# pmelchior/scarlet

Measured on AMD Instinct MI355X. Metric: PGM iters/sec over batched blends; achieved HBM GB/s vs roofline, higher is better.
Workload: dtype f32; 1 GPU; configs[2]: 1024 independent 5-band 128x128 blends in total, 10 ExtendedSource components (41x41) each, ConvolutionRenderer FFT 160x160; iterations 0..1234 of a fit from the initial parameters; loop=blend, blends_total=1024, components_per_blend=10, sub_ranges_per_gpu=3

## Files before the change

scarlet_amd/batch.py:

```python

import collections
import ctypes

import numpy as np

from . import _lib, operator


MonotonicPlanes = collections.namedtuple("MonotonicPlanes", "center_radius variance max_iter")
MonotonicPlanes.__doc__ = """The constraint of the coefficients of ``StarletMorphology(monotonic=True)`` as the device
runs it: ``MonotonicMaskConstraint((h // 2, w // 2), center_radius, variance, max_iter)`` on
every plane.  Given to ``ComponentSpec(starlet=(coefficients, MonotonicPlanes(...)))`` in the
place of the thresholds."""


def monotonic_planes_prox(stack, rule=MonotonicPlanes(1, 0.0, 3)):
    out = np.array(stack, dtype=np.float32, order="C")
    assert out.ndim == 3
    planes, h, w = out.shape
    _lib.check(_lib.load().smi_starlet_monotonic_mask_f32(
        _lib.ptr(out, ctypes.c_float), planes, h, w, int(rule.center_radius),
        float(rule.variance), int(rule.max_iter)))
    return out

# ... 547 lines not shown
        return a.value, e.value

    def states(self):
        out = np.zeros(self.n_blends, dtype=np.int32)
        _lib.check(self._lib.smi_batch_get_states(self._h, _lib.ptr(out, ctypes.c_int32)))
        return out

    def fit(self, max_iter=200, e_rel=1e-3, min_iter=1, prox_max_iter=10, sync_every=10):
        if max_iter > self.max_iter:
            raise ValueError("max_iter exceeds the loss-history capacity of this batch")
        n_iter = np.zeros(self.n_blends, dtype=np.int32)
        _lib.check(
            self._lib.smi_batch_fit(
                self._h, max_iter, e_rel, min_iter, prox_max_iter, sync_every,
                _lib.ptr(n_iter, ctypes.c_int32),
            )
        )
        loss = self.loss_history()
        last = np.array([loss[b][n_iter[b] - 1] if n_iter[b] else np.nan
                         for b in range(self.n_blends)])
        return n_iter, -last

    def loss_history(self):
        out = np.empty((self.n_blends, self.max_iter), dtype=np.float64)
        n = np.zeros(self.n_blends, dtype=np.int32)
        _lib.check(
            self._lib.smi_batch_get_loss(
                self._h, _lib.ptr(out, ctypes.c_double), self.max_iter,
                _lib.ptr(n, ctypes.c_int32),
            )
        )
        return [out[b, : min(n[b], self.max_iter)].copy() for b in range(self.n_blends)]

    def set_previous_loss(self, loss):
        loss = np.ascontiguousarray(np.broadcast_to(loss, (self.n_blends,)), dtype=np.float64)
        _lib.check(self._lib.smi_batch_set_previous_loss(self._h, _lib.ptr(loss, ctypes.c_double)))

    def add_observation(self, data, weights, kernel):
        data, weights, kernel = _lib.f32(data), _lib.f32(weights), _lib.f32(kernel)
        assert data.shape == weights.shape == (self.n_blends, self.C, self.H, self.W)
        assert kernel.shape == self._kernel_shape, "kernel stamp shape is fixed at construction"
        _lib.check(self._lib.smi_batch_add_observation(
            self._h, _lib.ptr(data, ctypes.c_float), _lib.ptr(weights, ctypes.c_float),
            _lib.ptr(kernel, ctypes.c_float)))

    def add_loss_constant(self, constant):
        c = np.ascontiguousarray(np.broadcast_to(constant, (self.n_blends,)), dtype=np.float64)
        _lib.check(self._lib.smi_batch_add_loss_constant(self._h, _lib.ptr(c, ctypes.c_double)))

    def set_sub_ranges(self, n):
        _lib.check(self._lib.smi_batch_set_sub_ranges(self._h, int(n)))

    def set_inline_render(self, on):
        _lib.check(self._lib.smi_batch_set_inline_render(self._h, int(bool(on))))

    def sub_ranges(self):
        n = ctypes.c_int32()
        _lib.check(self._lib.smi_batch_get_sub_ranges(self._h, ctypes.byref(n)))
        return n.value

    def attach_lowres(self, resampler, channels, data, weights, log_norm):
        channels = np.ascontiguousarray(channels, dtype=np.int32)
        data = np.ascontiguousarray(data, dtype=np.float32)
        weights = np.ascontiguousarray(weights, dtype=np.float32)
        assert data.shape == weights.shape and data.shape[0] == len(channels)
        self._lowres_shapes = getattr(self, "_lowres_shapes", []) + [data.shape]
        _lib.check(self._lib.smi_batch_attach_lowres(
            self._h, resampler, _lib.ptr(channels, ctypes.c_int32),
            _lib.ptr(data, ctypes.c_float), _lib.ptr(weights, ctypes.c_float), float(log_norm)))

    def lowres_rendered(self, index=0):
        out = np.empty(self._lowres_shapes[index], dtype=np.float32)
        _lib.check(self._lib.smi_batch_get_lowres_rendered(self._h, index,
                                                           _lib.ptr(out, ctypes.c_float)))
        return out

    def reset(self):
        _lib.check(self._lib.smi_batch_reset(self._h))

    def save_state(self):
        _lib.check(self._lib.smi_batch_save_state(self._h))

    def restore_state(self):
        _lib.check(self._lib.smi_batch_restore_state(self._h))

    def parameters(self):
        sed = np.empty((self.n_components, self.C), dtype=np.float32)
        morph = np.empty(int(self._morph_offsets[-1]), dtype=np.float32)
        _lib.check(
            self._lib.smi_batch_get_parameters(
                self._h, _lib.ptr(sed, ctypes.c_float), _lib.ptr(morph, ctypes.c_float)
            )
        )
        return sed, self._split_morphs(morph)

    def _split_starlets(self, flat):
        out, pos = [], 0
        for shape in self._star_shapes:
            n = int(np.prod(shape))
            out.append(flat[pos:pos + n].reshape(shape))
            pos += n
        return out

    def starlet_state(self, dtype=np.float32):
        n = int(sum(np.prod(s) for s in self._star_shapes))
        names = ("coeffs", "m", "v", "vhat", "gradient")
        bufs = [np.zeros(n, dtype=np.float32) for _ in names]
# ... 132 lines not shown
```

scarlet_amd/csrc/batch.hip:

```cpp
#include <rocfft/rocfft.h>

#include <algorithm>
#include <cmath>
#include <cstdlib>
#include <atomic>
#include <cstring>
#include <limits>
#include <map>
#include <mutex>
#include <thread>
#include <tuple>
#include <utility>

#include "common.h"

namespace smi {

static thread_local std::string g_error;
static std::atomic<int> g_hw_queues{4};
static std::atomic<long long> g_observation_uploads{0};
static std::mutex g_plan_mutex;
void set_error(const std::string &msg) { g_error = msg; }

static int next_fast_len(int n) {
// ... 101 lines not shown
    auto it = g_live_shapes.find(std::make_tuple(device, Fy, Fx));
    if (it != g_live_shapes.end() && --it->second <= 0) g_live_shapes.erase(it);
}

static int plans_get(int device, int Fy, int Fx, int count, bool shared, PlanPair *out) {
    if (!shared) return make_plans(Fy, Fx, count, out);
    std::lock_guard<std::mutex> guard(g_plan_mutex);
    PlanPair &p = g_plan_cache[device].by_count[count];
    if (!p.fwd) {
        const int rc = make_plans(Fy, Fx, count, &p);
        if (rc) return rc;
    }
    *out = p;
    return SMI_OK;
}

struct smi_batch {
    smi_batch_desc d{};
    int device = 0;
    hipStream_t stream = nullptr;
    bool null_renderer = false;
    bool fused = false;
    int Fy = 0, Fx = 0, Fxh = 0;
    int Py = 0, Px = 0;
    float2 *Kt = nullptr;
    long long *dbg = nullptr;
    float *P = nullptr, *Q = nullptr;
    float2 *S = nullptr, *Khat = nullptr;
    void *work = nullptr;
    rocfft_plan plan_fwd = nullptr, plan_inv = nullptr;
    bool plans_registered = false, plans_shared = false;
    rocfft_execution_info info = nullptr;
    float *data = nullptr, *weights = nullptr;
    float4 *dw = nullptr;
    bool own_obs = false;
    double *log_norm = nullptr;
    int32_t *comp_start = nullptr, *c_blend = nullptr, *c_oy = nullptr, *c_ox = nullptr,
            *c_h = nullptr, *c_w = nullptr, *c_flags = nullptr, *c_plan = nullptr;
    int64_t *c_moff = nullptr;
    float *c_sed_min_step = nullptr, *c_sed_rel = nullptr, *c_morph_step = nullptr,
          *c_morph_rel = nullptr, *c_min_grad = nullptr, *c_lthresh = nullptr;
    float *sed = nullptr, *morph = nullptr;
    float *mom[6] = {nullptr, nullptr, nullptr, nullptr, nullptr, nullptr};
    float *g_sed = nullptr, *g_morph = nullptr;
    float *xp_tmp = nullptr;
    int n_size_classes = 0;
    double *pt = nullptr, *g_center = nullptr;
    float *c_sigma = nullptr, *c_beta = nullptr;
    int n_point = 0;
    std::vector<double> box_center;
    std::vector<char> is_point;
    int n_shift = 0, max_box_side = 1, max_box_w = 1;
    float *shift_scratch = nullptr;
    bool inline_render = true;
    float *morph_param = nullptr, *c_shift_step = nullptr, *c_shift_rel = nullptr;
    int32_t *c_shift_fft = nullptr;
    std::vector<char> is_shift;
    smi::StarletView star{};
    int32_t *st_comp = nullptr, *st_planes = nullptr, *st_fixed = nullptr, *st_toff = nullptr;
    int64_t *st_coff = nullptr;
    float *st_thresh = nullptr, *st_coeffs = nullptr, *st_mom[3] = {nullptr, nullptr, nullptr},
          *st_grad = nullptr, *st_work = nullptr;
    int64_t n_star_coeffs = 0;
    int32_t *st_mono = nullptr, *st_mono_radius = nullptr, *st_mono_iter = nullptr;
    double *st_mono_var = nullptr;
    float *st_zsave = nullptr;
    smi::ProfileView prof{};
    int32_t *pf_comp = nullptr, *pf_kind = nullptr, *pf_fixed = nullptr;
    double *pf_step = nullptr, *pf_rel = nullptr, *pf_par = nullptr, *pf_grad = nullptr,
           *pf_mom[3] = {nullptr, nullptr, nullptr};
    std::vector<int64_t> h_moff;
    std::vector<int32_t> h_blend;
    float *c_center_floor = nullptr, *c_bg_level = nullptr, *c_fista_step = nullptr;
    float *c_sym_strength = nullptr;
    int32_t *c_chain_repeat = nullptr;
    int32_t mono_mask = 0;
    float *c_pos_floor = nullptr, *c_sed_floor = nullptr;
    double *fista_t = nullptr;
    smi::KernelShiftView ks{};
    float *ks_resid = nullptr;
    double2 *ks_tmp = nullptr;
    void *saved[12] = {};
    size_t saved_bytes[12] = {};
    int scheme = SMI_SCHEME_AMSGRAD;
    bool include_log_norm = true;
    bool lite_flags = false;
    int32_t *have_prev = nullptr;
    float *scratch = nullptr;
    int64_t n_morph = 0;
    bool have_components = false, have_obs = false, have_kernel = false;
    std::vector<smi::LowRes *> lowres;
    double *extra_terms = nullptr;
    int n_sub = 0;
    std::vector<int32_t> h_comp_start;
    struct ObsLayer {
        float *data = nullptr, *weights = nullptr;
        float2 *Kt = nullptr;
        float4 *dw = nullptr;
    };
    std::vector<ObsLayer> layers;
    float *Q2 = nullptr;
    int32_t *work_items = nullptr;
    int32_t stage_plan[kNumUpdateClasses];
    std::vector<int32_t> h_work_start;
    std::vector<hipStream_t> sub_streams;
    std::vector<hipEvent_t> sub_events;
    int32_t *state = nullptr, *zero_state = nullptr, *n_loss = nullptr, *status_out = nullptr;
    int32_t *it_base = nullptr;
    int32_t *frame_hw = nullptr;
    int32_t *pause_at = nullptr, *conv_flag = nullptr;
    std::vector<char> plan_shared;
    int32_t *h_round = nullptr;
    double *loss_hist = nullptr, *last_loss = nullptr, *loss_partial = nullptr;
    std::vector<SweepPlanDev> plans;
    SweepPlanDev *d_plans = nullptr;
    int max_levels = 0;
    BatchView view{};
    float b1 = 0.9f, b2 = 0.999f, eps = 1e-8f;
    double b1_f64 = 0.9, b2_f64 = 0.999;
    bool timing = false;
    std::vector<hipEvent_t> events;
    double phase_ms[6] = {0, 0, 0, 0, 0, 0};
    int timed_iters = 0;
};

namespace {

void refresh_view(smi_batch *b) {
    BatchView &v = b->view;
    v.nb = b->d.n_blends;
    v.C = b->d.C;
    v.H = b->d.H;
    v.W = b->d.W;
    v.Fy = b->Py;
    v.Fx = b->Px;
    v.n_comp = b->d.n_components;
    v.n_comp_total = b->d.n_components;
    v.comp_start = b->comp_start;
    v.c_blend = b->c_blend;
    v.c_oy = b->c_oy;
    v.c_ox = b->c_ox;
    v.c_h = b->c_h;
    v.c_w = b->c_w;
    v.c_flags = b->c_flags;
    v.c_plan = b->c_plan;
    v.c_moff = b->c_moff;
    v.c_sed_min_step = b->c_sed_min_step;
    v.c_sed_rel = b->c_sed_rel;
    v.c_morph_step = b->c_morph_step;
    v.c_morph_rel = b->c_morph_rel;
    v.c_min_grad = b->c_min_grad;
    v.c_lthresh = b->c_lthresh;
    v.sed = b->sed;
    v.morph = b->morph;
    v.m_sed = b->mom[0];
    v.v_sed = b->mom[1];
    v.vh_sed = b->mom[2];
    v.m_morph = b->mom[3];
    v.v_morph = b->mom[4];
    v.vh_morph = b->mom[5];
    v.data = b->data;
    v.weights = b->weights;
    v.dw = b->dw;
    v.it_base = b->it_base;
    v.frame_hw = b->frame_hw;
    v.pause_at = b->pause_at;
    v.conv_flag = b->conv_flag;
    v.log_norm = b->log_norm;
    v.state = b->state;
    v.n_loss = b->n_loss;
    v.loss_hist = b->loss_hist;
    v.hist_cap = b->d.max_iter;
    v.last_loss = b->last_loss;
    v.have_prev = b->have_prev;
    v.scratch = b->scratch;
    v.loss_partial = b->loss_partial;
    v.n_partial = b->fused ? b->d.C * (1 + (int)b->layers.size()) : (b->d.H * b->d.W + 255) / 256;
    v.plans = b->d_plans;
    v.max_levels = b->max_levels;
    v.fast_plans = 1;
    v.mono_mask = b->mono_mask;
    v.b1 = b->b1;
    v.b2 = b->b2;
    v.eps = b->eps;
    v.n_point = b->n_point;
    v.pt = b->pt;
    v.c_sigma = b->c_sigma;
    v.c_beta = b->c_beta;
    v.n_shift = b->n_shift;
    v.max_box_side = b->max_box_side;
    v.shift_scratch = b->shift_scratch;
    v.morph_param = b->morph_param;
    v.g_sed_buf = b->g_sed;
    v.g_morph_buf = b->g_morph;
    v.xp_tmp = b->xp_tmp;
    v.n_morph_total = b->n_morph;
    v.c_shift_step = b->c_shift_step;
    v.c_shift_rel = b->c_shift_rel;
    v.c_shift_fft = b->c_shift_fft;
    v.c_center_floor = b->c_center_floor;
    v.c_sym_strength = b->c_sym_strength;
    v.c_chain_repeat = b->c_chain_repeat;
    v.c_pos_floor = b->c_pos_floor;
    v.c_sed_floor = b->c_sed_floor;
    v.c_bg_level = b->c_bg_level;
    v.scheme = b->scheme;
    v.lite = b->scheme == SMI_SCHEME_FISTA || b->lite_flags;
    v.c_fista_step = b->c_fista_step;
    v.fista_t = b->fista_t;
    v.extra_term = b->extra_terms;
    v.n_extra = (int32_t)b->lowres.size();
    v.blend0 = 0;
    v.comp0 = 0;
    v.work = b->work_items;
    v.work0 = 0;
    v.work_start = b->h_work_start.data();
    v.nb_total = b->d.n_blends;
    for (int cls = 0; cls < kNumUpdateClasses; ++cls) {
        const int p = b->have_components ? b->stage_plan[cls] : -1;
        static const bool may_late = [] {
            const char *e = getenv("SMI_RING_LATE");
            return !e || atoi(e) != 0;
        }();
        const bool ok = p >= 0 && p < (int)b->plans.size() && b->plans[p].ring &&
                        kUpdateTeam[cls] == 64 && b->plans[p].ring_planes == 1 &&
                        (may_late || b->plans[p].ring_nat == b->plans[p].ring_pad);
        v.stage_plan[cls] = ok ? p : -1;
        v.stage_bytes[cls] = ok ? b->plans[p].ring_bytes : 0;
    }
    {
        const int slots = (b->max_box_w + 14) / 16 + 1;
        v.render_slots = slots <= 6 ? slots : 0;
    }
    for (const auto &pl : b->plans)
        if (!pl.slots) v.fast_plans = 0;
}

int ready(smi_batch *b) {
    SMI_REQUIRE(b != nullptr, "null batch");
    SMI_REQUIRE(b->have_components, "smi_batch_set_components has not been called");
    SMI_REQUIRE(b->have_obs, "smi_batch_set_observation has not been called");
    SMI_REQUIRE(b->null_renderer || b->have_kernel, "smi_batch_set_kernel has not been called");
    SMI_HIP(hipSetDevice(b->device));
    return SMI_OK;
}

int fft_exec(smi_batch *b, rocfft_plan plan, void *in, void *out) {
    void *ins[1] = {in}, *outs[1] = {out};
    SMI_FFT(rocfft_execute(plan, ins, outs, b->info));
    return SMI_OK;
}

int convolve(smi_batch *b, const BatchView &v, int conj) {
    if (b->null_renderer) return SMI_OK;
    if (b->fused) {
        set_error("internal: rocFFT convolution requested on the fused path");
        return SMI_ERR_INVALID;
    }
    int rc = fft_exec(b, b->plan_fwd, b->P, b->S);
    if (rc) return rc;
    launch_cmul(b->S, b->Khat, v.nb, v.C, (int64_t)b->Fy * b->Fxh, b->d.kernel_bands,
                b->d.kernel_per_blend, conj, v.state, b->stream);
    return fft_exec(b, b->plan_inv, b->S, b->Q);
}

BatchView unmasked_view(smi_batch *b) {
    BatchView v = b->view;
    v.state = b->zero_state;
    return v;
}

int upload_plans(smi_batch *b) {
    if (b->d_plans) {
        SMI_HIP(hipFree(b->d_plans));
        b->d_plans = nullptr;
    }
    if (!b->plans.empty()) {
        SMI_HIP(dev_alloc(&b->d_plans, b->plans.size()));
        SMI_HIP(hipMemcpy(b->d_plans, b->plans.data(), b->plans.size() * sizeof(SweepPlanDev),
                          hipMemcpyHostToDevice));
    }
    refresh_view(b);
    return SMI_OK;
}

// ... 2094 lines not shown
        }
    }
    SMI_HIP(hipGetLastError());
    return SMI_OK;
}

int smi_batch_gradient(smi_batch *b, float *g_sed, float *g_morph) {
    int rc = ready(b);
    if (rc) return rc;
    const BatchView v = unmasked_view(b);
    if (b->fused) {
        launch_render(v, b->P, b->stream);
        if ((rc = lowres_evaluate_all(b, 1))) return rc;
        if (b->ks.stamp && (rc = kernel_shift_backward(b, v, 0, 1))) return rc;
        if ((rc = launch_fused_conv(v, b->Fy, b->Fx, b->P, b->Kt, b->d.kernel_bands,
                                    b->d.kernel_per_blend, b->Q, 0, b->dbg, b->stream)))
            return rc;
        if ((rc = layers_evaluate(b, v, 1, b->stream))) return rc;
    } else {
        launch_render(v, b->P, b->stream);
        if ((rc = lowres_evaluate_all(b, 1))) return rc;
        if ((rc = convolve(b, v, 0))) return rc;
        launch_residual(v, b->Q, b->P, b->stream);
        if ((rc = convolve(b, v, 1))) return rc;
    }
    lowres_add_all(b);
    if ((rc = launch_update(v, b->Q, 0, 0.f, 0, b->g_sed, b->g_morph, 1, b->stream))) return rc;
    if ((rc = launch_point_sources(v, b->Q, 0, 0.f, 0, b->g_sed, b->g_center, 1, b->stream)))
        return rc;
    if ((rc = launch_shift_backward(v, b->Q, 0, b->g_center, 1, b->stream))) return rc;
    if ((rc = launch_starlet_step(v, b->star, b->Q, 0, 0.f, 0, 1, b->stream))) return rc;
    if ((rc = launch_profile_step(v, b->prof, b->Q, 0, 0.f, 0, 1, b->stream))) return rc;
    SMI_HIP(hipStreamSynchronize(b->stream));
    if (g_sed)
        SMI_HIP(hipMemcpy(g_sed, b->g_sed, (size_t)v.n_comp * v.C * sizeof(float),
                          hipMemcpyDeviceToHost));
    if (g_morph)
        SMI_HIP(hipMemcpy(g_morph, b->g_morph, (size_t)b->n_morph * sizeof(float),
                          hipMemcpyDeviceToHost));
    SMI_HIP(hipGetLastError());
    return SMI_OK;
}

static bool plain_batch(const smi_batch *b) {
    return b->fused && b->n_point == 0 && b->n_shift == 0 && b->star.n_star == 0 && b->prof.n_prof == 0 &&
           b->lowres.empty() && b->layers.empty() && !b->ks.stamp;
}

static bool inline_render(const smi_batch *b) {
    static const bool allowed = [] {
        const char *e = getenv("SMI_INLINE_RENDER");
        return !(e && e[0] == '0');
    }();
    return allowed && b->inline_render && b->fused && b->lowres.empty() && b->layers.empty() &&
           !b->ks.stamp && b->star.n_star == 0 && b->prof.n_prof == 0 && b->view.render_slots > 0;
}


static bool class_streams_pay(const smi_batch *b) {
    static const int forced = [] {
        const char *e = getenv("SMI_RANGE_CLASS_STREAMS");
        return e ? atoi(e) : -1;
    }();
    if (forced == 0 || b->n_size_classes < 2) return false;
    if (forced > 0) return true;
    return g_hw_queues.load(std::memory_order_relaxed) >= 8 && b->d.n_components >= 10000;
}

static int sub_ranges(const smi_batch *b) {
    if (!plain_batch(b)) return 1;
    const int nb = b->d.n_blends;
    const int queues = g_hw_queues.load(std::memory_order_relaxed);
    int n = b->n_sub > 0 ? b->n_sub : (nb < 128 ? 1 : (queues >= 8 && nb < 768) ? 4 : 3);
    if (b->n_sub <= 0 && class_streams_pay(b)) n = 2;
    return std::max(1, std::min(n, nb));
}

static int step_sub_ranges(smi_batch *b, int n_sub, int32_t it0, int32_t n_iter, float e_rel,
                           int32_t min_iter, int32_t prox_max_iter, int check) {
    int rc;
    while ((int)b->sub_streams.size() < n_sub - 1) {
        hipStream_t st;
        SMI_HIP(hipStreamCreateWithFlags(&st, hipStreamNonBlocking));
        b->sub_streams.push_back(st);
    }
    while ((int)b->sub_events.size() < n_sub) {
        hipEvent_t e;
        SMI_HIP(hipEventCreateWithFlags(&e, hipEventDisableTiming));
        b->sub_events.push_back(e);
    }
    const bool timing = b->timing;
    const bool no_cube = inline_render(b);
    if (timing) {
        const size_t need = (size_t)n_iter * 6;
        while (b->events.size() < need) {
            hipEvent_t e;
            SMI_HIP(hipEventCreate(&e));
            b->events.push_back(e);
        }
    }
    const int nb = b->d.n_blends;
    std::vector<BatchView> views(n_sub, b->view);
    for (int s = 0; s < n_sub; ++s) {
        const int lo = (int)((int64_t)s * nb / n_sub), hi = (int)((int64_t)(s + 1) * nb / n_sub);
        views[s].blend0 = lo;
        views[s].range_slot = s;
        views[s].nb = hi - lo;
// ... 95 lines not shown
            if (ev) SMI_HIP(hipEventRecord(ev[3], b->stream));
            if (ev) SMI_HIP(hipEventRecord(ev[4], b->stream));
        } else {
            launch_render(v, b->P, b->stream);
            if ((rc = lowres_evaluate_all(b, 1))) return rc;
            if (ev) SMI_HIP(hipEventRecord(ev[1], b->stream));
            if ((rc = convolve(b, v, 0))) return rc;
            if (ev) SMI_HIP(hipEventRecord(ev[2], b->stream));
            launch_residual(v, b->Q, b->P, b->stream);
            launch_finalize(v, it, e_rel, min_iter, check, b->stream);
            if (ev) SMI_HIP(hipEventRecord(ev[3], b->stream));
            if ((rc = convolve(b, v, 1))) return rc;
            if (ev) SMI_HIP(hipEventRecord(ev[4], b->stream));
        }
        lowres_add_all(b);
        if ((rc = launch_shift_backward(v, b->Q, it, nullptr, 0, b->stream))) return rc;
        b->star.b1 = b->b1_f64;
        b->star.b2 = b->b2_f64;
        if ((rc = launch_starlet_step(v, b->star, b->Q, it, e_rel, prox_max_iter, 0, b->stream)))
            return rc;
        if ((rc = launch_profile_step(v, b->prof, b->Q, it, e_rel, prox_max_iter, 0, b->stream)))
            return rc;
        if (plain) {
            if ((rc = launch_update_finalize(v, b->Q, it, e_rel, min_iter, check, prox_max_iter,
                                             b->stream)))
                return rc;
        } else if ((rc = launch_update(v, b->Q, it, e_rel, prox_max_iter, nullptr, nullptr, 0,
                                       b->stream))) {
            return rc;
        }
        if ((rc = launch_point_sources(v, b->Q, it, e_rel, prox_max_iter, nullptr, nullptr, 0,
                                       b->stream)))
            return rc;
        if ((rc = launch_shift_forward(v, 1, b->stream))) return rc;
        if ((rc = launch_starlet_forward(v, b->star, 1, b->stream))) return rc;
        if ((rc = launch_profile_forward(v, b->prof, 1, b->stream))) return rc;
        if (b->ks.stamp && (rc = refresh_shifted_kernel(b, 1))) return rc;
        if (check) launch_advance(v, b->stream);
        if (ev) SMI_HIP(hipEventRecord(ev[5], b->stream));
    }
    SMI_HIP(hipGetLastError());
    if (timing && n_iter > 0) return collect_phase_times(b, n_iter);
    return SMI_OK;
}

int smi_batch_set_sub_ranges(smi_batch *b, int32_t n) {
    SMI_REQUIRE(b && n >= 0, "bad argument");
    b->n_sub = n;
    return SMI_OK;
}

int smi_batch_set_inline_render(smi_batch *b, int32_t on) {
    SMI_REQUIRE(b != nullptr, "null batch");
    b->inline_render = on != 0;
    return SMI_OK;
}

int smi_batch_get_sub_ranges(smi_batch *b, int32_t *n) {
    SMI_REQUIRE(b && n, "null argument");
    *n = sub_ranges(b);
    return SMI_OK;
}

int smi_batch_status(smi_batch *b, int32_t *n_active, int32_t *first_error) {
    SMI_REQUIRE(b, "null batch");
    SMI_HIP(hipSetDevice(b->device));
    launch_count_active(b->state, b->d.n_blends, b->status_out, b->stream);
    int32_t out[2] = {0, -1};
    SMI_HIP(hipMemcpyAsync(out, b->status_out, sizeof(out), hipMemcpyDeviceToHost, b->stream));
    SMI_HIP(hipStreamSynchronize(b->stream));
    SMI_HIP(hipGetLastError());
    if (n_active) *n_active = out[0];
    if (first_error) *first_error = out[1];
    return SMI_OK;
}

int smi_batch_get_states(smi_batch *b, int32_t *state) {
    SMI_REQUIRE(b && state, "null argument");
    SMI_HIP(hipSetDevice(b->device));
    SMI_HIP(hipStreamSynchronize(b->stream));
    SMI_HIP(hipMemcpy(state, b->state, b->d.n_blends * sizeof(int32_t), hipMemcpyDeviceToHost));
    for (int32_t i = 0; i < b->d.n_blends; ++i) state[i] = std::min(state[i], 3);
    return SMI_OK;
}

int smi_batch_fit(smi_batch *b, int32_t max_iter, float e_rel, int32_t min_iter,
                  int32_t prox_max_iter, int32_t sync_every, int32_t *n_iter) {
    int rc = ready(b);
    if (rc) return rc;
    SMI_REQUIRE(max_iter >= 0, "negative max_iter");
    if (sync_every <= 0) sync_every = 10;
    int it = 0;
    while (it < max_iter) {
        const int chunk = std::min(sync_every, max_iter - it);
        if ((rc = smi_batch_step(b, it, chunk, e_rel, min_iter, prox_max_iter, 1))) return rc;
        it += chunk;
        int32_t active = 0, err = -1;
        if ((rc = smi_batch_status(b, &active, &err))) return rc;
        if (err >= 0) {
            set_error("blend " + std::to_string(err) + ": parameters are not finite");
            return SMI_ERR_ARITHMETIC;
        }
        if (active == 0) break;
    }
    if (n_iter) {
        SMI_HIP(hipMemcpy(n_iter, b->n_loss, b->d.n_blends * sizeof(int32_t), hipMemcpyDeviceToHost));
    }
// ... 194 lines not shown
```

scarlet_amd/csrc/common.h:

```cpp
#pragma once

#include <hip/hip_runtime.h>
#include <stdint.h>

#include <string>
#include <vector>

#include "../../include/scarlet_amd.h"

namespace smi {

void set_error(const std::string &msg);

#define SMI_HIP(expr)                                                              \
    do {                                                                           \
        hipError_t _e = (expr);                                                    \
        if (_e != hipSuccess) {                                                    \
            smi::set_error(std::string(#expr) + ": " + hipGetErrorString(_e));     \
            return SMI_ERR_HIP;                                                    \
        }                                                                          \
    } while (0)

#define SMI_REQUIRE(cond, msg)                                                     \
    do {                                                                           \
// ... 95 lines not shown
    const int32_t *c_blend, *c_oy, *c_ox, *c_h, *c_w, *c_flags, *c_plan;
    const int64_t *c_moff;
    const float *c_sed_min_step, *c_sed_rel, *c_morph_step, *c_morph_rel;
    const float *c_min_grad, *c_lthresh;
    float *sed, *morph;
    float *m_sed, *v_sed, *vh_sed, *m_morph, *v_morph, *vh_morph;
    const float *data, *weights;
    const float4 *dw;
    const double *log_norm;
    int32_t *state;
    int32_t *n_loss;
    double *loss_hist;
    int32_t hist_cap;
    double *last_loss;
    const int32_t *have_prev;
    double *loss_partial;
    int32_t n_partial;
    const SweepPlanDev *plans;
    int32_t max_box_pixels;
    int32_t max_levels;
    int32_t fast_plans;
    int32_t mono_mask;
    float b1, b2, eps;
    int32_t n_point;
    double *pt;
    const float *c_sigma;
    const float *c_beta;
    int32_t n_shift, max_box_side;
    float *shift_scratch;
    float *morph_param;
    float *g_sed_buf, *g_morph_buf;
    float *xp_tmp;
    int64_t n_morph_total;
    const float *c_shift_step;
    const float *c_shift_rel;
    const int32_t *c_shift_fft;
    const float *c_center_floor;
    const float *c_sym_strength;
    const float *c_pos_floor;
    const float *c_sed_floor = nullptr;
    const int32_t *c_chain_repeat;
    const float *c_bg_level;
    float *scratch;
    int32_t lite;
    int32_t scheme;
    const float *c_fista_step;
    double *fista_t;
    const double *extra_term;
    int32_t n_extra;
    int32_t blend0, comp0;
    const int32_t *work;
    int32_t work0;
    int32_t render_slots;
    const int32_t *work_start;
    int32_t nb_total;
    int32_t stage_plan[kNumUpdateClasses];
    uint32_t stage_bytes[kNumUpdateClasses];
    int32_t fail_code = 3;
    int32_t range_slot = 0;
    int32_t class_streams = 0;
    const int32_t *pause_at = nullptr;
    int32_t *conv_flag = nullptr;
    const int32_t *it_base = nullptr;
    const int32_t *frame_hw = nullptr;
    __device__ __forceinline__ int local_it(int b, int it) const {
        return it_base ? it - it_base[b] : it;
    }
    __device__ __forceinline__ int frame_h(int b) const { return frame_hw ? frame_hw[2 * b] : H; }
    __device__ __forceinline__ int frame_w(int b) const { return frame_hw ? frame_hw[2 * b + 1] : W; }
};

void launch_render(const BatchView &v, float *P, hipStream_t s);
void launch_residual(const BatchView &v, const float *Q, float *R, hipStream_t s);
void launch_finalize(const BatchView &v, int32_t it, float e_rel, int32_t min_iter,
                     int32_t check, hipStream_t s);
void launch_advance(const BatchView &v, hipStream_t s);
void launch_cmul(float2 *S, const float2 *K, int32_t nb, int32_t C, int64_t plane,
                 int32_t k_bands, int32_t k_per_blend, int32_t conj,
                 const int32_t *state, hipStream_t s);
int launch_update(const BatchView &v, const float *G, int32_t it, float e_rel,
                  int32_t prox_max_iter, float *g_sed_out, float *g_morph_out,
                  int32_t grad_only, hipStream_t s);
int launch_update_finalize(const BatchView &v, const float *G, int32_t it, float e_rel,
                           int32_t min_iter, int32_t check, int32_t prox_max_iter,
                           hipStream_t s);
int launch_point_sources(const BatchView &v, const float *G, int32_t it, float e_rel,
                         int32_t prox_max_iter, float *g_sed_out, double *g_center_out,
                         int32_t mode, hipStream_t s);
bool shift_needs_scratch(int max_box_pixels, int max_box_side);
int launch_shift_backward(const BatchView &v, const float *G, int32_t it, double *g_shift_out,
                          int32_t grad_only, hipStream_t s);
int launch_shift_forward(const BatchView &v, int32_t respect_state, hipStream_t s);

struct StarletView {
    int32_t n_star = 0;
    int32_t max_pixels = 0;
    const int32_t *comp = nullptr;
    const int32_t *planes = nullptr;
    const int32_t *fixed = nullptr;
    const int64_t *coff = nullptr;
    const int32_t *toff = nullptr;
    const float *thresh = nullptr;
    float *coeffs = nullptr, *m = nullptr, *v = nullptr, *vh = nullptr;
    float *grad = nullptr;
    float *work = nullptr;
    const int32_t *mono = nullptr;
// ... 127 lines not shown
```

scarlet_amd/csrc/fused_conv.hip:

```cpp
#include <cstdlib>
#include <type_traits>

#include "common.h"
#include "fft_regs.h"

namespace smi {

using fftk::cf;
using fftk::cmul;
using fftk::cmulc;
using fftk::ld;
using fftk::st;

namespace {

#ifndef SMI_CONV_THREADS
#define SMI_CONV_THREADS 1024
#endif
constexpr int kThreads = SMI_CONV_THREADS;
constexpr int kF2 = 16;

constexpr int conv_column_stride(int fy) { return ((fy + fy / kF2 + 3) / 8) * 8 + 4; }
constexpr size_t conv_lds_bytes(int fy, int fx) {
    return sizeof(float2) * ((size_t)(fx / 2) * conv_column_stride(fy) + 2 * fy + fx) +
// ... 389 lines not shown
        for (int m = 0; m < M; ++m) {
            uint32_t t = x4 + 64u * m;
            t = t < wlim4 ? t : kNone;
            mv[m].x = __builtin_bit_cast(float, __builtin_amdgcn_raw_buffer_load_b32(r, row0 + t, 0, 0));
            mv[m].y = __builtin_bit_cast(float, __builtin_amdgcn_raw_buffer_load_b32(r, row1 + t, 0, 0));
        }
        return none ? -1 : n1lo;
    }
    __device__ __forceinline__ void close(int n1lo_, float sd_, const cf (&mv)[M], cf (&acc)[FX1]) const {
        const cf sd = cf{sd_, sd_};
        fftk::static_for<0, NX1>([&](auto lo) {
            constexpr int n1lo = decltype(lo)::value;
            if (n1lo_ == n1lo) {
#pragma unroll
                for (int m = 0; m < M; ++m)
                    if (n1lo + m < NX1) acc[n1lo + m] = fftk::fma2(mv[m], sd, acc[n1lo + m]);
                asm volatile("; n1lo = %0" ::"n"(n1lo));
            }
        });
    }
    __device__ __forceinline__ void run(int b, int lane, cf (&acc)[FX1]) const {
#pragma unroll
        for (int n1 = 0; n1 < NX1; ++n1) acc[n1] = cf{0.f, 0.f};
        const int cs = v.comp_start[b], ce = v.comp_start[b + 1];
        for (int kb = cs; kb < ce; kb += 64) {
            const int kk = kb + lane;
            const bool have = kk < ce;
            Lanes l;
            l.oy = have ? v.c_oy[kk] : 0;
            l.ox = have ? v.c_ox[kk] : 0;
            l.h = have ? v.c_h[kk] : 0;
            l.w = have ? v.c_w[kk] : 0;
            l.mo = have ? (int)v.c_moff[kk] : 0;
            l.sd = have ? v.sed[kk * v.C + band_c] : 0.f;
            const bool hit = have && l.oy < ylo + 8 && l.oy + l.h > ylo && l.oy < H && l.ox < W &&
                             l.ox + l.w > 0;
            unsigned long long todo = __ballot(hit);
            if (!todo) continue;
            cf mva[M], mvb[M];
            float sda, sdb;
            int na = open(todo, l, sda, mva);
            for (;;) {
                const int nb = open(todo, l, sdb, mvb);
                close(na, sda, mva, acc);
                if (nb < 0) break;
                na = open(todo, l, sda, mva);
                close(nb, sdb, mvb, acc);
                if (na < 0) break;
            }
        }
    }
};

extern __shared__ __attribute__((aligned(16))) float2 lds_conv[];

template <int FY1, int FX1, int ZB, bool EXT>
__global__ __launch_bounds__(kThreads) void fused_conv_kernel(BatchView v, const float *model,
                                                              const float2 *Kt, int k_bands,
                                                              int k_per_blend, float *out,
                                                              int mode, long long *dbg) {
    using C = Cfg<FY1, FX1, ZB>;
    constexpr int NX1 = C::NX1;
    const int total = gridDim.x;
    int lid = blockIdx.x;
    if (total % 8 == 0) lid = (blockIdx.x % 8) * (total / 8) + blockIdx.x / 8;
    const int b = lid / v.C + v.blend0, c = lid % v.C;
    if (v.state[b] >= 2) return;
    const int tid = threadIdx.x;
    const int H = v.H, W = v.W;
    const int Hb = EXT ? v.frame_h(b) : H, Wb = EXT ? v.frame_w(b) : W;

    Conv<FY1, FX1, ZB> cv;
    cv.T = lds_conv;
    cv.twy = cv.T + C::NT * C::SY;
    cv.twx = cv.twy + C::FY;
    cv.tid = tid;
    cv.n_pairs = (H + 1) / 2;
    cv.first_block_item();
    cv.qtab = cv.twx + C::FX;
    double *loss_part = reinterpret_cast<double *>(cv.qtab + C::FY);
    const int64_t band = ((int64_t)b * v.C + c) * H * W;
    const int n_items = cv.stride_items();
    using Item = typename Conv<FY1, FX1, ZB>::StrideItem;

    const bool have_cube = model != nullptr;
    const plane_t r_model = band_plane(have_cube ? model + band : v.data + band, H * W);
    cf mrow[FX1];
    auto fetch_model = [&](const Item &s) {
        const PairRows a = pair_rows(2 * s.j, s.n2, W);
        fftk::static_for<0, NX1>([&](auto n1c) {
            constexpr int n1 = decltype(n1c)::value;
            mrow[n1] = pair_load<n1>(r_model, a);
        });
    };
    auto render_rows = [&](const Item &s) {
        const int j0 = __builtin_amdgcn_readfirstlane(s.j - ((tid & 63) >> 4));
        if (v.render_slots <= 4) {
            const ModelGather<FX1, NX1, 4> g{v, c, Hb, Wb, 2 * s.j, s.n2, 2 * j0};
            g.run(b, tid & 63, mrow);
        } else {
            const ModelGather<FX1, NX1, (FX1 < 6 ? FX1 : 6)> g{v, c, Hb, Wb, 2 * s.j, s.n2, 2 * j0};
            g.run(b, tid & 63, mrow);
        }
    };
    if (have_cube) fetch_model(cv.stride_item(tid));
    for (int j = tid; j < C::FY; j += kThreads) {
        float s, co;
        sincospif(2.0f * (float)((j / kF2) * (j % kF2)) / (float)C::FY, &s, &co);
        cv.twy[j] = make_float2(co, -s);
    }
    for (int j = tid; j < C::FX; j += kThreads) {
        float s, co;
        sincospif(2.0f * (float)((j / kF2) * (j % kF2)) / (float)C::FX, &s, &co);
        cv.twx[j] = make_float2(co, -s);
    }
    {
        const int y0 = 2 * cv.n_pairs, tail = kF2 * C::NY1 - y0;
        for (int i = tid; i < tail * C::NT; i += kThreads)
            cv.T[(i / tail) * C::SY + sk(y0 + i % tail)] = make_float2(0.f, 0.f);
    }
    const float2 *K = Kt + ((int64_t)(k_per_blend ? b : 0) * k_bands + (k_bands == 1 ? 0 : c)) *
                               C::FY * C::NKX;
    for (int j = tid; j < C::FY; j += kThreads) cv.qtab[j] = K[(int64_t)(C::FX / 2) * C::FY + j];
    __syncthreads();
#ifndef SMI_DBG_BLOCK
#define SMI_DBG_BLOCK 0
#endif
#define SMI_STAMP(i) if (dbg && tid == 0 && blockIdx.x == SMI_DBG_BLOCK) dbg[i] = clock64()
    SMI_STAMP(0);

    for (int it = tid; (have_cube ? it : it - (tid & 63)) < n_items; it += kThreads) {
        const Item s = cv.stride_item(it);
        if (have_cube) {
            if (it != tid) fetch_model(s);
#pragma unroll
            for (int n1 = 0; n1 < NX1; ++n1)
                if (kF2 * n1 + s.n2 >= W) mrow[n1] = cf{0.f, 0.f};
        } else {
            render_rows(s);
        }
        if (s.on) cv.stride_forward(mrow, s);
    }
    lds_barrier();
    SMI_STAMP(6);
    cv.blocks_forward();
    SMI_STAMP(1);
    cv.columns(K, false);
    SMI_STAMP(2);
    double loss = 0.0;
    {
        cf loss2 = cf{0.f, 0.f};
        const int64_t pband = ((int64_t)b * v.C + c) * cv.n_pairs * W;
        const char *p_dw = reinterpret_cast<const char *>(v.dw + pband);
        const plane_t r_rendered = band_plane(out + band, H * W);
#ifndef SMI_CONV_PRE
#define SMI_CONV_PRE 8
#endif
        constexpr int kPre = SMI_CONV_PRE < NX1 ? SMI_CONV_PRE : NX1;
        cf dv[NX1], wv[NX1];
        auto fetch = [&](const Item &s, auto from, auto to) {
            uint32_t o = (uint32_t)(min(s.j, cv.n_pairs - 1) * W + s.n2) * 16u;
            asm volatile("" : "+v"(o));
            fftk::static_for<decltype(from)::value, decltype(to)::value>([&](auto n1c) {
                constexpr int n1 = decltype(n1c)::value;
                dw_load<n1>(p_dw, o, dv[n1], wv[n1]);
            });
        };
        using std::integral_constant;
        const Item s0 = cv.stride_item(tid);
        fetch(s0, integral_constant<int, 0>{}, integral_constant<int, kPre>{});
        constexpr int kLate = NX1 > 8 ? NX1 - 8 : 0;
        cv.blocks_inverse([&] { fetch(s0, integral_constant<int, kPre>{}, integral_constant<int, NX1 - kLate>{}); });
        SMI_STAMP(10);
        for (int it = tid; it < n_items; it += kThreads) {
            const Item s = cv.stride_item(it);
            const int y = 2 * s.j;
            if (it != tid) fetch(s, integral_constant<int, 0>{}, integral_constant<int, NX1 - kLate>{});
            cf m[FX1];
            cv.stride_inverse(m, s);
            fetch(s, integral_constant<int, NX1 - kLate>{}, integral_constant<int, NX1>{});
#pragma unroll
            for (int n1 = 0; n1 < NX1; ++n1) {
                const int x = kF2 * n1 + s.n2;
// ... 61 lines not shown
    *k0 = make_float2(0.5f * (a.x + b.x), 0.5f * (a.y + b.y));
    *kn = make_float2(0.5f * (a.x - b.x), 0.5f * (a.y - b.y));
}

__global__ void stamp_dft_x(const float *kern, double2 *A, int ph, int pw, int Fx, int NKX) {
    const int img = blockIdx.y;
    const int i = blockIdx.x * blockDim.x + threadIdx.x;
    if (i >= ph * NKX) return;
    const int dy = i / NKX, kx = i - dy * NKX;
    double re = 0.0, im = 0.0;
    for (int dx = 0; dx < pw; ++dx) {
        int t = (kx * (dx - pw / 2)) % Fx;
        if (t < 0) t += Fx;
        double s, c;
        sincospi(2.0 * (double)t / (double)Fx, &s, &c);
        const double k = (double)kern[((int64_t)img * ph + dy) * pw + dx];
        re += k * c;
        im -= k * s;
    }
    A[(int64_t)img * ph * NKX + i] = make_double2(re, im);
}

template <int FY1>
__global__ void stamp_dft_y(const double2 *A, float2 *Kt, int ph, int NKX, double scale) {
    constexpr int FY = FY1 * kF2;
    const int img = blockIdx.y;
    const int i = blockIdx.x * blockDim.x + threadIdx.x;
    if (i >= FY * NKX) return;
    const int ky = i / NKX, kx = i - ky * NKX;
    double re = 0.0, im = 0.0;
    for (int dy = 0; dy < ph; ++dy) {
        int t = (ky * (dy - ph / 2)) % FY;
        if (t < 0) t += FY;
        double s, c;
        sincospi(2.0 * (double)t / (double)FY, &s, &c);
        const double2 a = A[((int64_t)img * ph + dy) * NKX + kx];
        re += a.x * c + a.y * s;
        im += a.y * c - a.x * s;
    }
    Kt[((int64_t)img * NKX + column_of(kx, 2 * (NKX - 1))) * FY + pos<FY1>(ky)] =
        make_float2((float)(re * scale), (float)(im * scale));
}

#endif

template <int FY1, int FX1, int ZB, bool EXT>
int launch_ext(const BatchView &v, const float *model, const float2 *Kt, int k_bands,
               int k_per_blend, float *out, int mode, long long *dbg, hipStream_t s) {
    using C = Cfg<FY1, FX1, ZB>;
    auto kern = fused_conv_kernel<FY1, FX1, ZB, EXT>;
    static size_t configured[kMaxDevices] = {};
    if (int rc = ensure_dynamic_lds(reinterpret_cast<const void *>(kern), C::lds_bytes, configured))
        return rc;
    hipLaunchKernelGGL(kern, dim3(v.nb * v.C), dim3(kThreads), C::lds_bytes, s, v, model, Kt,
                       k_bands, k_per_blend, out, mode, dbg);
    return SMI_OK;
}

template <int FY1, int FX1, int ZB>
int launch_zb(const BatchView &v, const float *model, const float2 *Kt, int k_bands,
              int k_per_blend, float *out, int mode, long long *dbg, hipStream_t s) {
    if (v.frame_hw)
        return launch_ext<FY1, FX1, ZB, true>(v, model, Kt, k_bands, k_per_blend, out, mode, dbg, s);
    return launch_ext<FY1, FX1, ZB, false>(v, model, Kt, k_bands, k_per_blend, out, mode, dbg, s);
}

template <int FY1, int FX1>
int launch_impl(const BatchView &v, const float *model, const float2 *Kt, int k_bands,
                int k_per_blend, float *out, int mode, long long *dbg, hipStream_t s) {
    const int zy = FY1 - (v.H + kF2 - 1) / kF2, zx = FX1 - (v.W + kF2 - 1) / kF2;
    const int zb = zy < zx ? zy : zx;
    if (zb >= 2) return launch_zb<FY1, FX1, 2>(v, model, Kt, k_bands, k_per_blend, out, mode, dbg, s);
    if (zb == 1) return launch_zb<FY1, FX1, 1>(v, model, Kt, k_bands, k_per_blend, out, mode, dbg, s);
    return launch_zb<FY1, FX1, 0>(v, model, Kt, k_bands, k_per_blend, out, mode, dbg, s);
}

}

#ifndef SMI_CONV_SHORT_ROWS
bool fused_conv_supported(int Fy, int Fx) {
    auto ok = [](int f) { return f == 64 || f == 80 || f == 96 || f == 128 || f == 160; };
    if (!ok(Fy) || !ok(Fx)) return false;
    return conv_lds_bytes(Fy, Fx) <= 160 * 1024;
}

int fused_conv_length(int n) {
    for (int f : {64, 80, 96, 128, 160})
        if (f >= n) return f;
    return 0;
}

#endif

#define SMI_FUSED_DISPATCH(FN, ...)                                             \
    switch (Fy / 16 * 100 + Fx / 16) {                                          \
        case 404: return FN<4, 4>(__VA_ARGS__);                  \
        case 405: return FN<4, 5>(__VA_ARGS__);                  \
        case 406: return FN<4, 6>(__VA_ARGS__);                  \
        case 408: return FN<4, 8>(__VA_ARGS__);                  \
        case 410: return FN<4, 10>(__VA_ARGS__);                 \
        case 504: return FN<5, 4>(__VA_ARGS__);                  \
        case 505: return FN<5, 5>(__VA_ARGS__);                  \
        case 506: return FN<5, 6>(__VA_ARGS__);                  \
        case 508: return FN<5, 8>(__VA_ARGS__);                  \
        case 510: return FN<5, 10>(__VA_ARGS__);                 \
        case 604: return FN<6, 4>(__VA_ARGS__);                  \
        case 605: return FN<6, 5>(__VA_ARGS__);                  \
// ... 95 lines not shown
```

Baseline: 1.402 million blend-iterations/s.

## Render blend model into an LDS frame before the FFT forward pass

Adds an LDS-resident frame renderer for the inline-render path. Components are scattered as sed times morph into a shared-memory image, with double-buffered unit loads, before the strided forward FFT reads rows from it. This replaces the per-row gather of all components and is meant to cut redundant global reads and per-item component scans. The cost is extra LDS barriers per tile. It reuses the FFT transpose buffer, so it is guarded by a fit check, a thread-count check and an env toggle, with mode 2 keeping the old gather.

```diff
diff --git a/scarlet_amd/batch.py b/scarlet_amd/batch.py
--- a/scarlet_amd/batch.py
+++ b/scarlet_amd/batch.py
@@ -623,7 +623,7 @@
         _lib.check(self._lib.smi_batch_set_sub_ranges(self._h, int(n)))
 
     def set_inline_render(self, on):
-        _lib.check(self._lib.smi_batch_set_inline_render(self._h, int(bool(on))))
+        _lib.check(self._lib.smi_batch_set_inline_render(self._h, 2 if int(on) == 2 else int(bool(on))))
 
     def sub_ranges(self):
         n = ctypes.c_int32()
diff --git a/scarlet_amd/csrc/batch.hip b/scarlet_amd/csrc/batch.hip
--- a/scarlet_amd/csrc/batch.hip
+++ b/scarlet_amd/csrc/batch.hip
@@ -177,7 +177,7 @@
     std::vector<char> is_point;
     int n_shift = 0, max_box_side = 1, max_box_w = 1;
     float *shift_scratch = nullptr;
-    bool inline_render = true;
+    int inline_render = 1;
     float *morph_param = nullptr, *c_shift_step = nullptr, *c_shift_rel = nullptr;
     int32_t *c_shift_fft = nullptr;
     std::vector<char> is_shift;
@@ -250,6 +250,14 @@
 };
 
 namespace {
+
+static int32_t render_lds(const smi_batch *b) {
+    static const bool allowed = [] {
+        const char *e = getenv("SMI_RENDER_LDS");
+        return !(e && e[0] == '0');
+    }();
+    return allowed && b->inline_render == 1;
+}
 
 void refresh_view(smi_batch *b) {
     BatchView &v = b->view;
@@ -356,6 +364,7 @@
     {
         const int slots = (b->max_box_w + 14) / 16 + 1;
         v.render_slots = slots <= 6 ? slots : 0;
+        v.render_lds = render_lds(b);
     }
     for (const auto &pl : b->plans)
         if (!pl.slots) v.fast_plans = 0;
@@ -2556,7 +2565,7 @@
         const char *e = getenv("SMI_INLINE_RENDER");
         return !(e && e[0] == '0');
     }();
-    return allowed && b->inline_render && b->fused && b->lowres.empty() && b->layers.empty() &&
+    return allowed && b->inline_render != 0 && b->fused && b->lowres.empty() && b->layers.empty() &&
            !b->ks.stamp && b->star.n_star == 0 && b->prof.n_prof == 0 && b->view.render_slots > 0;
 }
 
@@ -2758,7 +2767,9 @@
 
 int smi_batch_set_inline_render(smi_batch *b, int32_t on) {
     SMI_REQUIRE(b != nullptr, "null batch");
-    b->inline_render = on != 0;
+    SMI_REQUIRE(on >= 0 && on <= 2, "inline render: 0 (cube), 1 (default) or 2 (gather)");
+    b->inline_render = on;
+    b->view.render_lds = render_lds(b);
     return SMI_OK;
 }
 
diff --git a/scarlet_amd/csrc/common.h b/scarlet_amd/csrc/common.h
--- a/scarlet_amd/csrc/common.h
+++ b/scarlet_amd/csrc/common.h
@@ -171,6 +171,7 @@
     const int32_t *work;
     int32_t work0;
     int32_t render_slots;
+    int32_t render_lds = 1;
     const int32_t *work_start;
     int32_t nb_total;
     int32_t stage_plan[kNumUpdateClasses];
diff --git a/scarlet_amd/csrc/fused_conv.hip b/scarlet_amd/csrc/fused_conv.hip
--- a/scarlet_amd/csrc/fused_conv.hip
+++ b/scarlet_amd/csrc/fused_conv.hip
@@ -465,6 +465,128 @@
     }
 };
 
+template <int NX1>
+struct FrameRender {
+    static constexpr int kWaves = kThreads / 64, kRows = 48, RC = kRows / kWaves;
+    static constexpr uint32_t kNone = 0x40000000u;
+    static constexpr int kPitch = kF2 * NX1 + 8;
+    const BatchView &v;
+    float *img;
+    int band_c, H, W, wave, lane;
+    struct Lanes {
+        int oy, ox, h, w, mo;
+        float sd;
+    };
+    struct Unit {
+        int oy, ox, r0, c0, r1, c1;
+        float sd;
+        bool live;
+    };
+    Lanes l;
+    unsigned long long todo;
+    int row0, col0, kb;
+    Unit ua;
+    float mva[RC];
+
+    __device__ __forceinline__ void load_lanes(int b) {
+        const int ce = v.comp_start[b + 1], kk = kb + lane;
+        const bool have = kk < ce;
+        l.oy = have ? v.c_oy[kk] : 0;
+        l.ox = have ? v.c_ox[kk] : 0;
+        l.h = have ? v.c_h[kk] : 0;
+        l.w = have ? v.c_w[kk] : 0;
+        l.mo = have ? (int)v.c_moff[kk] : 0;
+        l.sd = have ? v.sed[kk * v.C + band_c] : 0.f;
+        const bool hit = have && l.oy < H && l.oy + l.h > 0 && l.ox < W && l.ox + l.w > 0;
+        todo = __ballot(hit);
+        row0 = col0 = 0;
+    }
+    __device__ __forceinline__ void open(Unit &u, float (&mv)[RC]) {
+        const bool none = todo == 0;
+        const int kl = none ? 0 : __builtin_ctzll(todo);
+        u.oy = __builtin_amdgcn_readlane(l.oy, kl);
+        u.ox = __builtin_amdgcn_readlane(l.ox, kl);
+        const int hh = __builtin_amdgcn_readlane(l.h, kl), w = __builtin_amdgcn_readlane(l.w, kl);
+        const float *mbase = v.morph + __builtin_amdgcn_readlane(l.mo, kl);
+        const plane_t r = band_plane(mbase, hh * w);
+        u.sd = __builtin_bit_cast(float, __builtin_amdgcn_readlane(__builtin_bit_cast(int, l.sd), kl));
+        u.live = !none;
+        const int rlo = max(0, -u.oy), rhi = min(hh, H - u.oy);
+        const int clo = max(0, -u.ox), chi = min(w, W - u.ox);
+        u.r0 = rlo + row0;
+        u.c0 = clo + col0;
+        u.r1 = none ? 0 : rhi;
+        u.c1 = chi;
+        col0 += 64;
+        if (u.c0 + 64 >= chi) {
+            col0 = 0;
+            row0 += kRows;
+            if (u.r0 + kRows >= rhi) {
+                row0 = 0;
+                todo &= todo - 1;
+            }
+        }
+        const int cx = u.c0 + lane;
+        const uint32_t x4 = cx < u.c1 ? 4u * (uint32_t)cx : kNone;
+#pragma unroll
+        for (int i = 0; i < RC; ++i) {
+            const int ry = u.r0 + wave + kWaves * i;
+            const uint32_t o = ry < u.r1 ? (uint32_t)(ry * w) * 4u + x4 : kNone;
+            mv[i] = __builtin_bit_cast(float, __builtin_amdgcn_raw_buffer_load_b32(r, o, 0, 0));
+        }
+    }
+    __device__ __forceinline__ void close(const Unit &u, const float (&mv)[RC]) const {
+        if (!u.live) return;
+        const int cx = u.c0 + lane;
+        float *p = img + (u.oy + u.r0 + wave) * kPitch + u.ox + cx;
+#pragma unroll
+        for (int i = 0; i < RC; ++i) {
+            if (cx < u.c1 && u.r0 + wave + kWaves * i < u.r1)
+                p[kWaves * i * kPitch] = fmaf(u.sd, mv[i], p[kWaves * i * kPitch]);
+        }
+        lds_barrier();
+    }
+    __device__ __forceinline__ void start(int b) {
+        kb = v.comp_start[b];
+        load_lanes(b);
+        open(ua, mva);
+    }
+    __device__ __forceinline__ void clear(int tid, int n_pairs) const {
+        float4 *q = reinterpret_cast<float4 *>(img);
+        for (int i = tid; i < 2 * n_pairs * (kPitch / 4); i += kThreads) q[i] = make_float4(0.f, 0.f, 0.f, 0.f);
+    }
+    __device__ __forceinline__ void finish(int b) {
+        const int ce = v.comp_start[b + 1];
+        for (;;) {
+            for (;;) {
+                Unit ub;
+                float mvb[RC];
+                open(ub, mvb);
+                close(ua, mva);
+                if (!ub.live) break;
+                open(ua, mva);
+                close(ub, mvb);
+                if (!ua.live) break;
+            }
+            kb += 64;
+            if (kb >= ce) break;
+            load_lanes(b);
+            open(ua, mva);
+        }
+    }
+    template <int FX1>
+    __device__ __forceinline__ void read_rows(int j, int n2, cf (&mrow)[FX1]) const {
+        const float *p = img + 2 * j * kPitch + n2;
+#pragma unroll
+        for (int n1 = 0; n1 < NX1; ++n1) mrow[n1] = cf{p[kF2 * n1], p[kPitch + kF2 * n1]};
+    }
+};
+
+constexpr bool frame_render_fits(int n_pairs, int nx1, int fy, int fx) {
+    return (size_t)2 * n_pairs * (kF2 * nx1 + 8) * sizeof(float) <=
+           sizeof(float2) * (size_t)(fx / 2) * conv_column_stride(fy);
+}
+
 extern __shared__ __attribute__((aligned(16))) float2 lds_conv[];
 
 template <int FY1, int FX1, int ZB, bool EXT>
@@ -516,7 +638,11 @@
             g.run(b, tid & 63, mrow);
         }
     };
+    const bool lds_frame = !have_cube && v.render_lds;
+    FrameRender<NX1> fr{v, reinterpret_cast<float *>(cv.T), c, Hb, Wb,
+                        __builtin_amdgcn_readfirstlane(tid >> 6), tid & 63};
     if (have_cube) fetch_model(cv.stride_item(tid));
+    if (lds_frame) fr.start(b);
     for (int j = tid; j < C::FY; j += kThreads) {
         float s, co;
         sincospif(2.0f * (float)((j / kF2) * (j % kF2)) / (float)C::FY, &s, &co);
@@ -527,11 +653,13 @@
         sincospif(2.0f * (float)((j / kF2) * (j % kF2)) / (float)C::FX, &s, &co);
         cv.twx[j] = make_float2(co, -s);
     }
-    {
+    auto zero_tail_rows = [&] {
         const int y0 = 2 * cv.n_pairs, tail = kF2 * C::NY1 - y0;
         for (int i = tid; i < tail * C::NT; i += kThreads)
             cv.T[(i / tail) * C::SY + sk(y0 + i % tail)] = make_float2(0.f, 0.f);
-    }
+    };
+    if (lds_frame) fr.clear(tid, cv.n_pairs);
+    else zero_tail_rows();
     const float2 *K = Kt + ((int64_t)(k_per_blend ? b : 0) * k_bands + (k_bands == 1 ? 0 : c)) *
                                C::FY * C::NKX;
     for (int j = tid; j < C::FY; j += kThreads) cv.qtab[j] = K[(int64_t)(C::FX / 2) * C::FY + j];
@@ -542,6 +670,14 @@
 #define SMI_STAMP(i) if (dbg && tid == 0 && blockIdx.x == SMI_DBG_BLOCK) dbg[i] = clock64()
     SMI_STAMP(0);
 
+    if (lds_frame) {
+        fr.finish(b);
+        const Item s = cv.stride_item(tid);
+        if (s.on) fr.read_rows(s.j, s.n2, mrow);
+        lds_barrier();
+        zero_tail_rows();
+        if (s.on) cv.stride_forward(mrow, s);
+    } else
     for (int it = tid; (have_cube ? it : it - (tid & 63)) < n_items; it += kThreads) {
         const Item s = cv.stride_item(it);
         if (have_cube) {
@@ -709,7 +845,11 @@
     static size_t configured[kMaxDevices] = {};
     if (int rc = ensure_dynamic_lds(reinterpret_cast<const void *>(kern), C::lds_bytes, configured))
         return rc;
-    hipLaunchKernelGGL(kern, dim3(v.nb * v.C), dim3(kThreads), C::lds_bytes, s, v, model, Kt,
+    BatchView w = v;
+    const int n_pairs = (v.H + 1) / 2;
+    w.render_lds = v.render_lds && !model && n_pairs * kF2 <= kThreads &&
+                   frame_render_fits(n_pairs, C::NX1, C::FY, C::FX);
+    hipLaunchKernelGGL(kern, dim3(v.nb * v.C), dim3(kThreads), C::lds_bytes, s, w, model, Kt,
                        k_bands, k_per_blend, out, mode, dbg);
     return SMI_OK;
 }
```

Result: slower. 1.235 million blend-iterations/s (-12.0%).
